# ChainSafe/lumenos

Measured on AMD Instinct MI355X. Metric: prove_eval_seconds_16384x4096, lower is better.
Workload: dtype u64; 1 GPU; Encode+Commit+InnerProduct(r,b)+QueryCols 16384x4096 LogN=14 L=12 K=2 rhoInv=2 queries=309; parallelism=1 GPU: the whole job resident in HBM

## Files before the change

### lumenos_amd/csrc/lm_common.h

```cpp
#pragma once
#include <hip/hip_runtime.h>

#include <algorithm>
#include <cstdarg>
#include <cstdint>
#include <cstdio>
#include <map>
#include <memory>
#include <mutex>
#include <set>
#include <string>
#include <utility>
#include <vector>

#include "../../include/lumenos_hip.h"
#include "lm_arith.h"
#include "lm_dev.h"

#define LM_MAX_LIMBS LUMEN_MAX_LIMBS

struct lm_modmap {
    uint32_t period;
    uint8_t idx[LM_MAX_LIMBS];
};

struct lm_mods {
    mod_t m[LM_MAX_LIMBS];
};

struct lm_prof_entry {
    double total_ms = 0;
    uint64_t launches = 0;
    uint64_t units = 0;
};

struct lm_galois_key {
    lm_dev<u64> d_key;
    lm_dev<uint32_t> d_index;
    lm_dev<uint32_t> d_inv_index;
};

struct lumen_set {
    uint32_t count = 0;
    uint32_t nl = 0;
    uint32_t logw = 0;
    u64 *d = nullptr;
    size_t words = 0;
    bool owner = true;
    lumen_ctx *home = nullptr;
};

struct lm_shared {
    std::recursive_mutex mu;
    lm_dev<tw_t> tw_fwd;
    lm_dev<tw_t> tw_inv;
    std::vector<uint64_t> roots;
    uint32_t fieldN = 0;
    lm_dev<tw_t> scal;
    std::map<uint64_t, lm_galois_key> gkeys;
    std::map<std::string, std::shared_ptr<void>> ext;
};

struct lm_tuning {
    uint32_t ks_batch = 64;
    uint32_t ks_lanes = 0;
    int32_t ks_fused_digits = -1;
    uint32_t debug = 0;
    uint32_t modup_tgroup = 3, moddown_tgroup = 1;
    uint32_t ks_placement = 6;
    uint32_t batch_chunks = 0;
    uint32_t rccl_shared_device = 0;
};

struct lumen_ctx {
    lm_tuning tune;
    std::recursive_mutex mu;
    std::shared_ptr<lm_shared> sh;
    int device = 0;
    hipStream_t stream = nullptr;
    hipStream_t stream2 = nullptr;
    hipEvent_t ev_fork = nullptr, ev_join = nullptr;
    hipStream_t stream_aux = nullptr;
    hipEvent_t ev_aux = nullptr;
    hipEvent_t ev_xdep = nullptr;
    uint32_t aux_digests = 0;
    const u64 *aux_lo = nullptr, *aux_hi = nullptr;
    uint8_t *aux_host = nullptr;
    size_t aux_host_cap = 0;
    void *stage_host = nullptr;
    size_t stage_cap = 0;
    hipEvent_t ev_stage = nullptr;
    void *io_host[2] = {nullptr, nullptr};
    hipEvent_t ev_io[2] = {nullptr, nullptr};
    uint32_t logN = 0, N = 0, L = 0, K = 0;
    uint64_t T = 0;
    uint64_t mod[LM_MAX_LIMBS] = {0};
    uint64_t psi[LM_MAX_LIMBS] = {0};
    lm_mods mods;
    tw_t ninv[LM_MAX_LIMBS];
    std::vector<uint64_t> &roots;
    uint32_t &fieldN;
    std::map<uint64_t, lm_galois_key> &gkeys;
    std::map<std::string, std::shared_ptr<void>> &ext;
    uint64_t mul_counter = 0;
    std::map<std::string, lm_dev<unsigned char>> scratch;
    struct pool_block {
        void *p;
        hipEvent_t ready;
    };
    std::multimap<size_t, pool_block> pool;
    size_t pool_bytes = 0;
    std::set<const void *> lds_attr_done;
    bool prof = false;
    std::map<std::string, lm_prof_entry> prof_tab;
    struct pending_ev {
        std::string name;
        hipEvent_t a, b;
        uint64_t units;
    };
    std::vector<pending_ev> prof_pending;
    std::vector<hipEvent_t> ev_pool;
    hipEvent_t tm0 = nullptr, tm1 = nullptr;
    std::string err;
    explicit lumen_ctx(std::shared_ptr<lm_shared> s)
        : sh(std::move(s)), roots(sh->roots), fieldN(sh->fieldN), gkeys(sh->gkeys), ext(sh->ext) {}
};

static inline size_t lm_ctw(const lumen_ctx *ctx, const lumen_set *s);
#define LM_FULL_WIDTH(ctx, set, what) \
    LM_CHECK(ctx, (set)->logw == 0, "%s: lane-sharded set (1/%u of every limb) where a full-width set is required", what, 1u << (set)->logw)

#define LM_ENTER(ctx)                                             \
    std::lock_guard<std::recursive_mutex> lm_lock_((ctx)->mu);    \
    (void)hipSetDevice((ctx)->device);                            \
    (void)hipGetLastError()
#define LM_SHARED_LOCK(ctx) std::lock_guard<std::recursive_mutex> lm_shlock_((ctx)->sh->mu)

template <class T>
static inline std::shared_ptr<T> lm_ext_get(lumen_ctx *ctx, const std::string &key) {
    LM_SHARED_LOCK(ctx);
    auto it = ctx->ext.find(key);
    return it == ctx->ext.end() ? std::shared_ptr<T>() : std::static_pointer_cast<T>(it->second);
}
static inline void lm_ext_put(lumen_ctx *ctx, const std::string &key, std::shared_ptr<void> v) {
    LM_SHARED_LOCK(ctx);
    ctx->ext[key] = std::move(v);
}

static inline size_t lm_ctw(const lumen_ctx *ctx, const lumen_set *s) { return (size_t)2 * s->nl * (ctx->N >> s->logw); }
// ... 22 lines not shown

template <class... P, class... A>
static inline int lm_launch_flat(lumen_ctx *ctx, void (*kernel)(P...), size_t threads, A &&...args) {
    hipLaunchKernelGGL(kernel, dim3((uint32_t)((threads + 255) / 256)), dim3(256), 0, ctx->stream, std::forward<A>(args)...);
    LM_HIP(ctx, hipGetLastError());
    return 0;
}

struct lm_set_guard {
    lumen_ctx *ctx;
    lumen_set *s;
    lm_set_guard(lumen_ctx *c, lumen_set *x) : ctx(c), s(x) {}
    ~lm_set_guard() {
        if (s) lumen_set_destroy(ctx, s);
    }
    lumen_set *release() {
        lumen_set *r = s;
        s = nullptr;
        return r;
    }
    lm_set_guard(const lm_set_guard &) = delete;
    lm_set_guard &operator=(const lm_set_guard &) = delete;
};

void lm_set_release_async(lumen_ctx *ctx, lumen_set *set);

void *lm_scratch(lumen_ctx *ctx, const char *name, size_t bytes);
void lm_scratch_adopt(lumen_ctx *ctx, const char *name, void *p, size_t bytes);

struct lm_prof_scope {
    lumen_ctx *ctx;
    const char *name;
    uint64_t units;
    hipEvent_t a = nullptr;
    lm_prof_scope(lumen_ctx *c, const char *n, uint64_t u);
    ~lm_prof_scope();
};
void lm_prof_resolve(lumen_ctx *ctx);

static inline uint64_t h_mulmod(uint64_t a, uint64_t b, uint64_t q) {
    return (uint64_t)(((u128)a * b) % q);
}
static inline uint64_t h_powmod(uint64_t a, uint64_t e, uint64_t q) {
    uint64_t r = 1 % q;
    a %= q;
    while (e) {
        if (e & 1) r = h_mulmod(r, a, q);
        a = h_mulmod(a, a, q);
        e >>= 1;
    }
    return r;
}
static inline uint64_t h_invmod(uint64_t a, uint64_t q) { return h_powmod(a, q - 2, q); }
static inline tw_t h_tw(uint64_t w, uint64_t q) {
    tw_t t;
    t.w = w;
    t.wp = (u64)((((u128)w) << 64) / q);
    return t;
}
static inline uint64_t h_r64_mod(uint64_t q) { return (uint64_t)((((u128)1) << 64) % q); }
static inline uint64_t h_p_mod(const lumen_ctx *ctx, uint64_t q) {
    uint64_t P = 1 % q;
    for (uint32_t a = 0; a < ctx->K; a++) P = h_mulmod(P, ctx->mod[ctx->L + a] % q, q);
    return P;
}
static inline uint32_t h_bitrev(uint32_t x, int bits) {
    uint32_t r = 0;
    for (int i = 0; i < bits; i++) r = (r << 1) | ((x >> i) & 1);
    return r;
}

int lm_launch_ntt(lumen_ctx *ctx, u64 *d, uint32_t npoly, const lm_modmap &map, bool inverse);
struct lm_ninv_t;
int lm_launch_ntt_strided(lumen_ctx *ctx, const u64 *src, size_t src_poly_stride, u64 *dst,
                          size_t dst_poly_stride, uint32_t npoly, const lm_modmap &map, bool inverse,
                          const char *prof_name, const lm_ninv_t *inv_scale = nullptr);
int lm_launch_ntt_subring(lumen_ctx *ctx, uint32_t logn, const tw_t *tw, tw_t ninv_scale, const u64 *src,
                          size_t src_poly_stride, u64 *dst, size_t dst_poly_stride, uint32_t npoly,
                          uint32_t mod_idx, bool inverse, const mod_t *explicit_mod = nullptr);
mod_t lm_make_mod(uint64_t q);
void lm_build_tw(uint64_t q, uint64_t psi, uint32_t logN, std::vector<tw_t> &fwd, std::vector<tw_t> &inv);
int lm_rescale_polys(lumen_ctx *ctx, const u64 *src, uint32_t nl, u64 *dst, uint32_t target,
                     uint32_t npoly, u64 *work, u64 *tbuf);
lm_modmap lm_map_q(uint32_t nl);
lm_modmap lm_map_p(const lumen_ctx *ctx);
int lm_encode_dev(lumen_ctx *ctx, const lumen_set *matrix, const u64 *dzero, uint32_t rho_inv, lumen_set **encoded);
hipEvent_t lm_ev_get(lumen_ctx *ctx);
```

### lumenos_amd/csrc/lm_ctx.hip

```cpp
#include <cstring>
#include <thread>

#include "lm_ntt_dev.h"

thread_local std::string lm_global_err;

int lm_fail(lumen_ctx *ctx, const char *fmt, ...) {
    char buf[1024];
    va_list ap;
    va_start(ap, fmt);
    vsnprintf(buf, sizeof(buf), fmt, ap);
    va_end(ap);
    if (ctx) ctx->err = buf;
    lm_global_err = buf;
    fprintf(stderr, "[lumenos_hip] error: %s\n", buf);
    return 1;
}

void *lm_scratch(lumen_ctx *ctx, const char *name, size_t bytes) {
    auto &e = ctx->scratch[name];
    if (e && e.count() >= bytes) return e.get();
    if (e) lm_sync_all(ctx);
    return e.alloc(ctx, bytes, name) ? nullptr : e.get();
}
// ... 71 lines not shown
        }
        ctx->ev_pool.push_back(p.a);
        ctx->ev_pool.push_back(p.b);
    }
    ctx->prof_pending.clear();
}

lm_modmap lm_map_q(uint32_t nl) {
    lm_modmap m;
    m.period = nl;
    for (uint32_t i = 0; i < LM_MAX_LIMBS; i++) m.idx[i] = (uint8_t)(i < nl ? i : 0);
    return m;
}

lm_modmap lm_map_p(const lumen_ctx *ctx) {
    lm_modmap m;
    m.period = ctx->K;
    for (uint32_t i = 0; i < LM_MAX_LIMBS; i++) m.idx[i] = (uint8_t)(ctx->L + (i < ctx->K ? i : 0));
    return m;
}

mod_t lm_make_mod(uint64_t q) {
    mod_t m;
    m.q = q;
    m.qinv64 = (u64)((((u128)1) << 64) / q);
    u64 inv = 1;
    for (int it = 0; it < 6; it++) inv *= 2 - (u64)q * inv;
    m.qneg = (u64)0 - inv;
    u64 r = h_r64_mod(q);
    m.r2 = h_mulmod(r, r, q);
    return m;
}

void lm_build_tw(uint64_t q, uint64_t psi, uint32_t logN, std::vector<tw_t> &fwd, std::vector<tw_t> &inv) {
    uint32_t N = 1u << logN;
    fwd.resize(N);
    inv.resize(N);
    uint64_t psi_inv = h_invmod(psi, q), cf = 1, cb = 1;
    for (uint32_t j = 0; j < N; j++) {
        uint32_t r = h_bitrev(j, (int)logN);
        fwd[r] = h_tw(cf, q);
        inv[r] = h_tw(cb, q);
        cf = h_mulmod(cf, psi, q);
        cb = h_mulmod(cb, psi_inv, q);
    }
}

static void pool_drain(lumen_ctx *ctx) {
    for (auto &kv : ctx->pool) {
        hipFree(kv.second.p);
        if (kv.second.ready) ctx->ev_pool.push_back(kv.second.ready);
    }
    ctx->pool.clear();
    ctx->pool_bytes = 0;
}

static int ctx_private_init(lumen_ctx *ctx) {
    LM_HIP(ctx, hipSetDevice(ctx->device));
    LM_HIP(ctx, hipStreamCreate(&ctx->stream));
    LM_HIP(ctx, hipStreamCreate(&ctx->stream2));
    LM_HIP(ctx, hipEventCreateWithFlags(&ctx->ev_fork, hipEventDisableTiming));
    LM_HIP(ctx, hipEventCreateWithFlags(&ctx->ev_join, hipEventDisableTiming));
    LM_HIP(ctx, hipStreamCreate(&ctx->stream_aux));
    LM_HIP(ctx, hipEventCreateWithFlags(&ctx->ev_aux, hipEventDisableTiming));
    LM_HIP(ctx, hipEventCreateWithFlags(&ctx->ev_stage, hipEventDisableTiming));
    LM_HIP(ctx, hipEventCreateWithFlags(&ctx->ev_xdep, hipEventDisableTiming));
    LM_HIP(ctx, hipEventCreate(&ctx->tm0));
    LM_HIP(ctx, hipEventCreate(&ctx->tm1));
    return 0;
}

static int tuning_set(lm_tuning &t, const char *name, long v) {
    const std::string n(name ? name : "");
    auto in = [&](long lo, long hi) { return v >= lo && v <= hi; };
    if (n == "LUMEN_KS_BATCH") {
        if (!in(1, 4096)) return 2;
        t.ks_batch = (uint32_t)v;
    } else if (n == "LUMEN_KS_LANES") {
        if (!in(0, 2)) return 2;
        t.ks_lanes = (uint32_t)v;
    } else if (n == "LUMEN_KS_FUSED_DIGITS") {
        if (v > LM_MAX_LIMBS) return 2;
        t.ks_fused_digits = v >= 0 ? (int32_t)v : -1;
    } else if (n == "LUMEN_DEBUG") {
        t.debug = v != 0;
    } else if (n == "LUMEN_MODUP_TGROUP") {
        if (!in(1, 31)) return 2;
        t.modup_tgroup = (uint32_t)v;
    } else if (n == "LUMEN_MODDOWN_TGROUP") {
        if (!in(1, 31)) return 2;
        t.moddown_tgroup = (uint32_t)v;
    } else if (n == "LUMEN_KS_PLACEMENT") {
        if (!in(0, 32)) return 2;
        t.ks_placement = (uint32_t)v;
    } else if (n == "LUMEN_BATCH_CHUNKS") {
        if (!in(0, 4096)) return 2;
        t.batch_chunks = (uint32_t)v;
    } else {
        return 1;
    }
    return 0;
}
static void tuning_from_env(lm_tuning &t) {
    for (const char *n : {"LUMEN_KS_BATCH", "LUMEN_KS_LANES", "LUMEN_KS_FUSED_DIGITS", "LUMEN_DEBUG",
                          "LUMEN_MODUP_TGROUP", "LUMEN_MODDOWN_TGROUP", "LUMEN_KS_PLACEMENT", "LUMEN_BATCH_CHUNKS"}) {
        const char *e = getenv(n);
        if (e && *e && tuning_set(t, n, atol(e)))
            fprintf(stderr, "[lumenos_hip] %s=%s is out of range: ignored\n", n, e);
    }
}

extern "C" int lumen_ctx_set_tuning(lumen_ctx *ctx, const char *name, long value) {
    LM_CHECK(nullptr, ctx && name, "lumen_ctx_set_tuning: NULL argument");
    LM_ENTER(ctx);
    const int rc = tuning_set(ctx->tune, name, value);
    LM_CHECK(ctx, rc != 1, "unknown tuning switch %s", name);
    LM_CHECK(ctx, rc == 0, "tuning switch %s: value %ld is out of range (nothing changed)", name, value);
    return 0;
}

extern "C" int lumen_test_allow_shared_device_rccl(lumen_ctx *ctx, int on) {
    LM_CHECK(nullptr, ctx, "lumen_test_allow_shared_device_rccl: NULL ctx");
    LM_ENTER(ctx);
    ctx->tune.rccl_shared_device = on != 0;
    return 0;
}

extern "C" int lumen_ctx_wait(lumen_ctx *ctx, lumen_ctx *other) {
    LM_CHECK(nullptr, ctx && other, "lumen_ctx_wait: NULL argument");
    if (ctx == other) return 0;
    hipEvent_t ev;
    {
        LM_ENTER(other);
        LM_HIP(other, hipEventRecord(other->ev_xdep, other->stream));
        ev = other->ev_xdep;
    }
    LM_ENTER(ctx);
    LM_CHECK(ctx, ctx->device == other->device, "lumen_ctx_wait: contexts on devices %d and %d", ctx->device, other->device);
    LM_HIP(ctx, hipStreamWaitEvent(ctx->stream, ev, 0));
    return 0;
}

extern "C" int lumen_ctx_create(const lumen_params_desc *desc, lumen_ctx **out) {
    if (!desc || !out) return lm_fail(nullptr, "lumen_ctx_create: NULL argument");
    *out = nullptr;
    LM_CHECK(nullptr, desc->abi_version == LUMEN_ABI_VERSION, "ABI version mismatch: got %u want %u",
             desc->abi_version, LUMEN_ABI_VERSION);
    LM_CHECK(nullptr, lm_logn_supported(desc->log_n),
             "log_n %u unsupported: kernels are instantiated for N = 2^8 and 2^10..2^14", desc->log_n);
    LM_CHECK(nullptr, desc->num_q >= 1 && desc->num_q + desc->num_p <= LM_MAX_LIMBS,
             "bad limb counts L=%u K=%u", desc->num_q, desc->num_p);
    int ndev = 0;
    if (hipGetDeviceCount(&ndev) != hipSuccess || ndev == 0)
        return lm_fail(nullptr, "no HIP device visible: the lumenos HIP path has no CPU fallback");
    LM_CHECK(nullptr, desc->device >= 0 && desc->device < ndev, "device %d out of range (have %d)",
             desc->device, ndev);
    std::unique_ptr<lumen_ctx, void (*)(lumen_ctx *)> guard(new lumen_ctx(std::make_shared<lm_shared>()),
                                                            lumen_ctx_destroy);
    lumen_ctx *ctx = guard.get();
    tuning_from_env(ctx->tune);
    ctx->device = desc->device;
    ctx->logN = desc->log_n;
    ctx->N = 1u << desc->log_n;
    ctx->L = desc->num_q;
    ctx->K = desc->num_p;
    ctx->T = desc->plaintext_modulus;
    uint32_t LK = ctx->L + ctx->K, N = ctx->N;
    uint64_t two_n = 2ull * N;
    for (uint32_t i = 0; i < LK; i++) {
        uint64_t q = desc->moduli[i], psi = desc->psi[i];
        static_assert(3 * 0 + 8 >= 8, "the modulus bound (3 log_n + 8) q < 2^64 must imply 8 q < 2^64");
        const uint64_t qmax = UINT64_MAX / (3ull * desc->log_n + 8);
        if (q < (1ull << 20) || q > qmax || (q & (two_n - 1)) != 1)
            return lm_fail(nullptr, "modulus %u (%llu) must be == 1 mod 2N and below %llu", i,
                           (unsigned long long)q, (unsigned long long)qmax);
        if (h_powmod(psi, N, q) != q - 1)
            return lm_fail(nullptr, "psi[%u] is not a primitive 2N-th root of unity", i);
        ctx->mod[i] = q;
        ctx->psi[i] = psi;
        ctx->mods.m[i] = lm_make_mod(q);
        ctx->ninv[i] = h_tw(h_invmod(N % q, q), q);
    }
    for (uint32_t i = LK; i < LM_MAX_LIMBS; i++) ctx->mods.m[i] = ctx->mods.m[0];
    if (int rc = ctx_private_init(ctx)) return rc;
    std::vector<tw_t> f, b, fwd, inv;
    for (uint32_t i = 0; i < LK; i++) {
        lm_build_tw(ctx->mod[i], ctx->psi[i], ctx->logN, f, b);
// ... 469 lines not shown
```

### lumenos_amd/csrc/lm_keyswitch.hip

```cpp
#include <cstdlib>
#include <cstring>

#include "lm_ks_host.h"

uint32_t ks_batch(const lumen_ctx *ctx) { return ctx->tune.ks_batch; }

uint32_t ks_lanes(const lumen_ctx *ctx) {
    return ctx->tune.ks_lanes ? ctx->tune.ks_lanes : (ctx->logN <= 13 ? 2 : 1);
}

int check_level_of_chain(lumen_ctx *ctx, const lumen_set *in, const char *what) {
    LM_FULL_WIDTH(ctx, in, what);
    LM_CHECK(ctx, in->nl >= 1 && in->nl <= ctx->L, "%s: set has %u limbs, the chain has %u", what, in->nl, ctx->L);
    return 0;
}

__device__ __forceinline__ u32 bx_v(u128 A, u128 M, u64 y0, u64 y1, u64 m0, u64 m1) {
    const u128 D1 = A >= M ? A - M : M - A, D2 = 2 * M - A;
    if ((u64)(D1 >> 64) >= 8 && (u64)(D2 >> 64) >= 8) return A >= M ? 1u : 0u;
    double vf = 0.0;
    vf += (double)y0 / (double)m0;
    vf += (double)y1 / (double)m1;
    return (u32)(u64)vf;
}
// ... 565 lines not shown
    return 0;
}

static int modup_work_list(lumen_ctx *ctx, KsTables *tb, uint32_t B, const uint32_t **out) {
    const uint32_t LM_MODUP_TGROUP = ctx->tune.modup_tgroup;
    LM_SHARED_LOCK(ctx);
    LM_CHECK(ctx, B >= 1 && B <= 65535 && tb->beta <= 255 && tb->nl + ctx->K <= 255,
             "key-switch batch of %u columns (beta %u) does not fit the packed work list", B, tb->beta);
    const uint32_t cache_key = B | (LM_MODUP_TGROUP << 16);
    auto it = tb->d_work.find(cache_key);
    if (it != tb->d_work.end()) {
        *out = it->second.get();
        return 0;
    }
    const uint32_t LK = tb->nl + ctx->K, beta = tb->beta;
    std::vector<std::vector<uint8_t>> need(beta);
    for (uint16_t pr : tb->pairs) need[pr & 0xFF].push_back((uint8_t)(pr >> 8));
    std::vector<std::vector<uint32_t>> lists(8);
    for (uint32_t x = 0; x < 8; x++)
        for (uint32_t t0 = 0; t0 < LK; t0 += LM_MODUP_TGROUP)
            for (uint32_t b = x; b < B; b += 8)
                for (uint32_t d = 0; d < beta; d++)
                    for (uint8_t t : need[d])
                        if (t >= t0 && t < t0 + LM_MODUP_TGROUP) lists[x].push_back(b | (d << 16) | ((uint32_t)t << 24));
    return interleave_work_lists(ctx, lists, (size_t)B * tb->pairs.size(), "extension", tb->d_work, cache_key, out);
}

static int moddown_work_list(lumen_ctx *ctx, KsTables *tb, uint32_t B, const uint32_t **out) {
    const uint32_t LM_MODDOWN_TGROUP = ctx->tune.moddown_tgroup;
    LM_SHARED_LOCK(ctx);
    LM_CHECK(ctx, B >= 1 && 2 * (uint64_t)B <= 65535, "key-switch batch of %u columns does not fit the packed work list", B);
    const uint32_t cache_key = B | (LM_MODDOWN_TGROUP << 17);
    auto it = tb->d_work_down.find(cache_key);
    if (it != tb->d_work_down.end()) {
        *out = it->second.get();
        return 0;
    }
    const uint32_t L = tb->nl;
    std::vector<std::vector<uint32_t>> lists(8);
    for (uint32_t x = 0; x < 8; x++)
        for (uint32_t t0 = 0; t0 < L; t0 += LM_MODDOWN_TGROUP)
            for (uint32_t pw = x; pw < 2 * B; pw += 8)
                for (uint32_t t = t0; t < std::min<uint32_t>(t0 + LM_MODDOWN_TGROUP, L); t++) lists[x].push_back(pw | (t << 16));
    return interleave_work_lists(ctx, lists, (size_t)2 * B * L, "ModDown", tb->d_work_down, cache_key, out);
}

template <int LOGN>
static uint32_t intt_pack_slots(lumen_ctx *ctx) {
    static const uint32_t v = [&] {
        hipDeviceProp_t prop;
        int per_cu = 0;
        if (hipGetDeviceProperties(&prop, ctx->device) != hipSuccess) return 256u;
        (void)hipFuncSetAttribute(reinterpret_cast<const void *>(&k_intt_pack<LOGN>),
                                  hipFuncAttributeMaxDynamicSharedMemorySize, 160 * 1024);
        constexpr lm_geom g = lm_geom_lds(LOGN);
        if (hipOccupancyMaxActiveBlocksPerMultiprocessor(&per_cu, k_intt_pack<LOGN>, g.threads, g.lds) != hipSuccess || per_cu < 1) {
            per_cu = (int)std::max<size_t>(1, std::min<size_t>(160 * 1024 / g.lds, 2048 / g.threads));
        }
        (void)hipGetLastError();
        if (ctx->tune.debug)
            fprintf(stderr, "[lumenos_hip] k_intt_pack<%d>: %d workgroup(s) per CU, %d CUs\n", LOGN, per_cu,
                    prop.multiProcessorCount);
        return (uint32_t)prop.multiProcessorCount * (uint32_t)per_cu;
    }();
    return v;
}
static uint32_t ks_fused_digits(lumen_ctx *ctx, uint32_t B, uint32_t L) {
    const long forced = ctx->tune.ks_fused_digits;
    const uint32_t pairs = L / 2;
    if (forced >= 0) return std::min<uint32_t>((uint32_t)forced, pairs);
    uint32_t slots = 0;
    if (lm_for_logn(ctx, ctx->logN, [&](auto n) { return slots = intt_pack_slots<n>(ctx), 0; })) return 0;
    for (uint32_t nf = pairs; nf >= 1; nf--)
        if (((uint64_t)B * nf) % slots == 0) return nf;
    return 0;
}

static dim3 ks_mac_grid(const lumen_ctx *ctx, uint32_t B, uint32_t L) {
    return dim3(((ctx->N / LM_MAC_VEC + 255) / 256) * (L + ctx->K) * ((B + LM_MAC_COLS - 1) / LM_MAC_COLS));
}

}

int rotate_accumulate(lumen_ctx *ctx, const u64 *acc, u64 *acc_out, uint32_t B, const lm_galois_key &gk,
                      KsTables *tb, const KsScratch &s) {
    const uint32_t N = ctx->N, L = tb->nl, K = ctx->K, beta = tb->beta;
    const uint32_t pshift = ctx->L - L, key_beta = (ctx->L + K - 1) / K;
    const uint32_t nf = K == 2 ? ks_fused_digits(ctx, B, L) : 0;
    if (nf) {
        const uint32_t grid = B * nf + B * (L - 2 * nf);
        lm_prof_scope ps(ctx, "ks_intt_c1", (uint64_t)B * L);
        if (int rc = lm_for_logn(ctx, ctx->logN, [&](auto n) {
                return lm_launch(ctx, k_intt_pack<n>, lm_geom_lds(n), grid, acc, s.coef, B, L, nf, ctx->mods, tb->yscale,
                                 ctx->sh->tw_inv.get());
            }))
            return rc;
    } else {
        if (int rc = lm_launch_ntt_strided(ctx, acc + (size_t)L * N, (size_t)2 * L * N, s.coef, (size_t)L * N, B,
                                           lm_map_q(L), true, "ks_intt_c1", &tb->yscale))
            return rc;
    }
    if (K == 2 && nf < beta) {
        lm_prof_scope ps(ctx, "ks_pack_v", (uint64_t)B);
        hipLaunchKernelGGL(k_pack_v, dim3(2048), dim3(256), 0, ctx->stream, s.coef + (size_t)2 * nf * N, (size_t)L * N,
                           B, beta - nf, K, 2 * nf, L - 2 * nf, ctx->logN, ctx->mods);
        LM_HIP(ctx, hipGetLastError());
    }
    {
        const uint64_t nb = (uint64_t)B * tb->pairs.size();
        const uint32_t *work = nullptr;
        if (int rc = modup_work_list(ctx, tb, B, &work)) return rc;
        lm_prof_scope ps(ctx, "ks_modup_ntt", nb);
        if (int rc = lm_for_logn(ctx, ctx->logN, [&](auto n) {
                return lm_launch(ctx, k_modup_ntt<n>, lm_geom_fwd(n), (uint32_t)nb, s.coef, acc, s.ext, tb->d_bx.get(), B, L, K, beta,
                                 pshift, work, ctx->mods, ctx->sh->tw_fwd.get());
            }))
            return rc;
    }
    {
        lm_prof_scope ps(ctx, "ks_mac", (uint64_t)B);
        hipLaunchKernelGGL(k_ks_mac, ks_mac_grid(ctx, B, L), dim3(256), 0, ctx->stream, s.ext, acc, gk.d_key.get(), s.u, B, L, K,
                           beta, pshift, key_beta, ctx->logN, ctx->mods);
        LM_HIP(ctx, hipGetLastError());
    }
    {
        u64 *up = s.u + ks_u_at(0, L, B, L, K) * N;
        const size_t pstride = (size_t)K * N;
        if (int rc = lm_launch_ntt_strided(ctx, up, pstride, up, pstride, B * 2, lm_map_p(ctx), true, "ks_intt_p",
                                           &tb->yscale))
            return rc;
        if (K == 2) {
            lm_prof_scope ps(ctx, "ks_pack_v", (uint64_t)B);
            hipLaunchKernelGGL(k_pack_v, dim3(2048), dim3(256), 0, ctx->stream, up, pstride, B * 2, 1u, K, ctx->L, K,
                               ctx->logN, ctx->mods);
            LM_HIP(ctx, hipGetLastError());
        }
    }
    {
        const uint32_t *work_down = nullptr;
        if (int rc = moddown_work_list(ctx, tb, B, &work_down)) return rc;
        lm_prof_scope ps(ctx, "ks_moddown_ntt", (uint64_t)B * 2 * L);
        return lm_for_logn(ctx, ctx->logN, [&](auto n) {
            return lm_launch(ctx, k_moddown_ntt<n>, lm_geom_fwd(n), B * 2 * L, s.u, acc, acc_out, tb->d_bxp.get(), tb->d_pinv.get(),
                             gk.d_index.get(), gk.d_inv_index.get(), work_down, B, L, K, ctx->mods, ctx->sh->tw_fwd.get());
        });
    }
}

namespace {

int inner_sum_batch(lumen_ctx *ctx, u64 *acc, uint32_t B, uint32_t n, KsTables *tb, const KsScratch &s) {
    uint64_t gal[64];
    const uint32_t cnt = lumen_inner_sum_galois_elements(ctx, n, gal);
    for (uint32_t r = 0; r < cnt; r++) {
        const lm_galois_key *gk;
        {
            LM_SHARED_LOCK(ctx);
            auto it = ctx->gkeys.find(gal[r]);
            LM_CHECK(ctx, it != ctx->gkeys.end(), "Galois key for element %llu not loaded",
                     (unsigned long long)gal[r]);
            gk = &it->second;
        }
        u64 *src = (r & 1) ? s.acc2 : acc, *dst = (r & 1) ? acc : s.acc2;
        if (int rc = rotate_accumulate(ctx, src, dst, B, *gk, tb, s)) return rc;
    }
    if (cnt & 1)
        LM_HIP(ctx, hipMemcpyAsync(acc, s.acc2, (size_t)B * 2 * tb->nl * ctx->N * 8, hipMemcpyDeviceToDevice,
                                   ctx->stream));
    return 0;
}

}

extern "C" int lumen_ks_mac_probe(lumen_ctx *ctx, uint32_t batch, const void *ext, const void *acc, const void *key,
                                  void *u, uint32_t reps, float *ms_per_launch) {
    LM_CHECK(nullptr, ctx && ms_per_launch, "lumen_ks_mac_probe: NULL argument");
    LM_ENTER(ctx);
    KsTables *tb = nullptr;
    if (int rc = get_tables(ctx, &tb)) return rc;
    const uint32_t N = ctx->N, L = ctx->L, K = ctx->K, B = batch ? batch : ks_batch(ctx);
    LM_CHECK(ctx, B <= 65535 && reps >= 1 && reps <= 100000, "lumen_ks_mac_probe: batch %u / reps %u out of range", B, reps);
    KsScratch s;
    if (int rc = get_scratch(ctx, B, tb, &s)) return rc;
    if (!acc) acc = lm_scratch(ctx, "ks_acc", (size_t)B * 2 * L * N * 8);
    if (!acc) return 1;
    if (!key) {
        LM_SHARED_LOCK(ctx);
        LM_CHECK(ctx, !ctx->gkeys.empty(), "lumen_ks_mac_probe: no Galois key loaded");
        key = ctx->gkeys.begin()->second.d_key.get();
    }
    const u64 *pe = ext ? (const u64 *)ext : s.ext;
    u64 *pu = u ? (u64 *)u : s.u;
    const dim3 grid = ks_mac_grid(ctx, B, L);
    auto launch = [&] {
        hipLaunchKernelGGL(k_ks_mac, grid, dim3(256), 0, ctx->stream, pe, (const u64 *)acc, (const u64 *)key, pu, B, L, K,
                           tb->beta, 0u, tb->beta, ctx->logN, ctx->mods);
    };
    for (int i = 0; i < 3; i++) launch();
    LM_HIP(ctx, hipGetLastError());
    LM_HIP(ctx, hipEventRecord(ctx->tm0, ctx->stream));
    for (uint32_t i = 0; i < reps; i++) launch();
    LM_HIP(ctx, hipGetLastError());
    LM_HIP(ctx, hipEventRecord(ctx->tm1, ctx->stream));
    LM_HIP(ctx, hipEventSynchronize(ctx->tm1));
    float ms = 0;
    LM_HIP(ctx, hipEventElapsedTime(&ms, ctx->tm0, ctx->tm1));
    *ms_per_launch = ms / (float)reps;
    return 0;
}

static int check_inner_sum_level(lumen_ctx *ctx, const lumen_set *in, const char *what) {
    LM_FULL_WIDTH(ctx, in, what);
    LM_CHECK(ctx, in->nl == ctx->L, "%s is implemented at the top level only (set has %u of %u limbs)", what,
             in->nl, ctx->L);
    return 0;
}

namespace {

int inner_sum_at(lumen_ctx *ctx, const lumen_set *in, uint32_t n, lumen_set **out) {
    LM_CHECK(ctx, n && !(n & (n - 1)) && n <= ctx->N, "InnerSum length %u is not a power of two <= N", n);
    KsTables *top = nullptr, *tb = nullptr;
    if (int rc = get_tables(ctx, &top)) return rc;
    if (int rc = get_tables_at(ctx, in->nl, &tb)) return rc;
    lumen_set *o = nullptr;
    if (int rc = lumen_set_create(ctx, in->count, in->nl, &o)) return rc;
    lm_set_guard og(ctx, o);
    if (in->words)
        LM_HIP(ctx, hipMemcpyAsync(o->d, in->d, in->words * 8, hipMemcpyDeviceToDevice, ctx->stream));
    const uint32_t Bmax = std::min<uint32_t>(ks_batch(ctx), std::max(in->count, 1u));
    KsScratch s;
    if (int rc = get_scratch(ctx, Bmax, top, &s)) return rc;
    const size_t ctw = (size_t)2 * in->nl * ctx->N;
    for (uint32_t first = 0; first < in->count; first += Bmax) {
        const uint32_t B = std::min(Bmax, in->count - first);
        if (int rc = inner_sum_batch(ctx, o->d + (size_t)first * ctw, B, n, tb, s)) return rc;
    }
    if (int rc = acc_canon(ctx, o->d, o->words, in->nl)) return rc;
    *out = og.release();
    return 0;
}

int matrix_inner_sum_at(lumen_ctx *ctx, const lumen_set *matrix, const uint64_t *pt, uint32_t rows, lumen_set **out) {
    LM_CHECK(ctx, rows && !(rows & (rows - 1)) && rows <= ctx->N, "rows=%u is not a power of two <= N", rows);
    KsTables *top = nullptr, *tb = nullptr;
    if (int rc = get_tables(ctx, &top)) return rc;
    if (int rc = get_tables_at(ctx, matrix->nl, &tb)) return rc;
    u64 *ptT = nullptr;
    if (int rc = upload_ptT(ctx, pt, matrix->nl, &ptT)) return rc;
    const uint32_t N = ctx->N, L = matrix->nl;
    const uint32_t target = std::min<uint32_t>(2, L);
    lumen_set *o = nullptr;
    if (int rc = lumen_set_create(ctx, matrix->count, target, &o)) return rc;
    lm_set_guard og(ctx, o);
    const uint32_t Bmax = std::min<uint32_t>(ks_batch(ctx), std::max(matrix->count, 1u));
    const uint32_t group = std::min<uint32_t>(8 * Bmax, std::max(matrix->count, 1u));
    KsScratch s[2];
    const size_t ctw = (size_t)2 * L * N, octw = (size_t)2 * target * N;
    const size_t group_bytes = (size_t)group * 2 * ctx->L * N * 8;
    u64 *acc = nullptr;
    if (get_scratch(ctx, Bmax, top, &s[0], 0, &acc, group_bytes) || (ks_lanes(ctx) > 1 && get_scratch(ctx, Bmax, top, &s[1], 1)))
        return 1;
    u64 *work = (u64 *)lm_scratch(ctx, "rescale_work", group_bytes);
    u64 *tbuf = (u64 *)lm_scratch(ctx, "rescale_t", (size_t)group * 2 * N * 8);
    if (!acc || !work || !tbuf) return 1;
    for (uint32_t g0 = 0; g0 < matrix->count; g0 += group) {
        const uint32_t gn = std::min(group, matrix->count - g0);
        if (ks_lanes(ctx) > 1) {
            LM_HIP(ctx, hipEventRecord(ctx->ev_fork, ctx->stream));
            LM_HIP(ctx, hipStreamWaitEvent(ctx->stream2, ctx->ev_fork, 0));
        }
        uint32_t lane = 0;
        for (uint32_t first = 0; first < gn; first += Bmax, lane = (lane + 1) % ks_lanes(ctx)) {
            const uint32_t B = std::min(Bmax, gn - first);
            u64 *a = acc + (size_t)first * ctw;
            LaneGuard guard(ctx, (int)lane);
            if (int rc = launch_mul_plain(ctx, matrix->d + (size_t)(g0 + first) * ctw, a, ptT, (size_t)B * ctw, L, B))
                return rc;
            if (int rc = inner_sum_batch(ctx, a, B, rows, tb, s[lane])) return rc;
        }
        if (ks_lanes(ctx) > 1) {
            LM_HIP(ctx, hipEventRecord(ctx->ev_join, ctx->stream2));
            LM_HIP(ctx, hipStreamWaitEvent(ctx->stream, ctx->ev_join, 0));
        }
        if (L > target) {
            if (int rc = lm_rescale_polys(ctx, acc, L, o->d + (size_t)g0 * octw, target, gn * 2, work, tbuf)) return rc;
        } else {
            if (int rc = acc_canon(ctx, acc, (size_t)gn * ctw, L)) return rc;
            LM_HIP(ctx, hipMemcpyAsync(o->d + (size_t)g0 * octw, acc, (size_t)gn * ctw * 8, hipMemcpyDeviceToDevice,
                                       ctx->stream));
        }
    }
    *out = og.release();
    return 0;
}

}

extern "C" int lumen_inner_sum(lumen_ctx *ctx, const lumen_set *in, uint32_t n, lumen_set **out) {
    LM_CHECK(nullptr, ctx && in && out, "lumen_inner_sum: NULL argument");
    LM_ENTER(ctx);
    if (int rc = check_inner_sum_level(ctx, in, "InnerSum")) return rc;
    return inner_sum_at(ctx, in, n, out);
}

extern "C" int lumen_inner_sum_at_level(lumen_ctx *ctx, const lumen_set *in, uint32_t n, lumen_set **out) {
    LM_CHECK(nullptr, ctx && in && out, "lumen_inner_sum_at_level: NULL argument");
    LM_ENTER(ctx);
    if (int rc = check_level_of_chain(ctx, in, "InnerSum")) return rc;
    return inner_sum_at(ctx, in, n, out);
}

extern "C" int lumen_matrix_inner_sum(lumen_ctx *ctx, const lumen_set *matrix, const uint64_t *pt,
                                      uint32_t rows, lumen_set **out) {
    LM_CHECK(nullptr, ctx && matrix && pt && out, "lumen_matrix_inner_sum: NULL argument");
    LM_ENTER(ctx);
    if (int rc = check_inner_sum_level(ctx, matrix, "matrixInnerSumEval")) return rc;
    return matrix_inner_sum_at(ctx, matrix, pt, rows, out);
}

extern "C" int lumen_matrix_inner_sum_at_level(lumen_ctx *ctx, const lumen_set *matrix, const uint64_t *pt,
                                               uint32_t rows, lumen_set **out) {
    LM_CHECK(nullptr, ctx && matrix && pt && out, "lumen_matrix_inner_sum_at_level: NULL argument");
    LM_ENTER(ctx);
    if (int rc = check_level_of_chain(ctx, matrix, "matrixInnerSumEval")) return rc;
    return matrix_inner_sum_at(ctx, matrix, pt, rows, out);
}
```

### lumenos_amd/csrc/lm_ks_host.h

```cpp
#pragma once
#include "lm_ks_dev.h"

struct KsTables {
    lm_dev<bx_t> d_bx;
    lm_dev<bx_t> d_bxp;
    lm_dev<tw_t> d_pinv;
    uint32_t nl = 0;
    uint32_t beta = 0;
    lm_ninv_t yscale;
    std::vector<uint16_t> pairs;
    std::map<uint32_t, lm_dev<uint32_t>> d_work;
    std::map<uint32_t, lm_dev<uint32_t>> d_work_down;
};
int get_tables(lumen_ctx *ctx, KsTables **out);
int get_tables_at(lumen_ctx *ctx, uint32_t nl, KsTables **out);

struct KsScratch {
    u64 *coef, *ext, *u, *acc2;
};

int rotate_accumulate(lumen_ctx *ctx, const u64 *acc, u64 *acc_out, uint32_t B, const lm_galois_key &gk,
                      KsTables *tb, const KsScratch &s);
int get_scratch(lumen_ctx *ctx, uint32_t B, KsTables *tb, KsScratch *s, int lane = 0, u64 **group_acc = nullptr,
                size_t group_acc_bytes = 0);

int upload_ptT(lumen_ctx *ctx, const uint64_t *pt, uint32_t nl, u64 **out);
int launch_mul_plain(lumen_ctx *ctx, const u64 *ct, u64 *out, const u64 *ptT, size_t words, uint32_t nl,
                     uint32_t ncts);

std::shared_ptr<lm_galois_key> lm_relin_key(lumen_ctx *ctx);
int check_level_of_chain(lumen_ctx *ctx, const lumen_set *in, const char *what);
uint32_t ks_batch(const lumen_ctx *ctx);
uint32_t ks_lanes(const lumen_ctx *ctx);
struct LaneGuard {
    lumen_ctx *ctx;
    hipStream_t saved;
    LaneGuard(lumen_ctx *c, int lane) : ctx(c), saved(c->stream) {
        if (lane) ctx->stream = ctx->stream2;
    }
    ~LaneGuard() { ctx->stream = saved; }
};
```

### lumenos_amd/csrc/lm_rescale.hip

```cpp
#include "lm_ntt_dev.h"

struct rescale_consts {
    u64 half;
    u64 half_mod[LM_MAX_LIMBS];
    tw_t qlinv[LM_MAX_LIMBS];
};

template <int LOGN>
__global__ LM_GEOM_BOUNDS(lm_geom_lds(LOGN)) void k_rescale_last(const u64 *__restrict__ src, size_t src_poly_stride,
                                                       uint32_t last, u64 *__restrict__ tbuf, mod_t md,
                                                       tw_t ninv, u64 half, const tw_t *__restrict__ tw) {
    extern __shared__ __attribute__((aligned(16))) u64 sm[];
    constexpr uint32_t N = 1u << LOGN;
    const uint32_t tid = threadIdx.x;
    const lm_qc c = lm_make_qc(md);
    const u64 *p = src + (size_t)blockIdx.x * src_poly_stride + (size_t)last * N;
    u64 *o = tbuf + (size_t)blockIdx.x * N;
    auto ld = [&](uint32_t i0, u64 *v, int count) { lm_load_run(p, i0, v, count); };
    auto st = [&](uint32_t i, u64 v) { o[i] = lm_addmod(lm_shoup_cs(v, ninv, c.q, c.nq), half, c.q); };
    lm_ntt_inverse<LOGN>(sm, tw, c, tid, ld, st);
}

template <int LOGN>
__global__ LM_GEOM_BOUNDS(lm_geom_lds(LOGN)) void k_rescale_limb(const u64 *src, size_t src_poly_stride, u64 *dst,
// ... 16 lines not shown
        lm_load_run(cin, i0, cv, count);
#pragma unroll
        for (int k = 0; k < 8; k++)
            if (k < count) r[k] = lm_shoup_cs(lm_submod(cv[k], lm_reduce_s(v[k], c.q, c.nq, c.qinv64), c.q), qlinv, c.q, c.nq);
        lm_store_run(o, i0, r, count);
    };
    lm_ntt_forward<LOGN>(sm, tw_all + (size_t)limb * N, c, tid, ld, st);
}

struct rs_step_t {
    u64 k;
    u64 pad;
    tw_t inv;
};
struct rs_half_t {
    u64 h[LM_MAX_LIMBS];
};
struct RescaleTables {
    lm_dev<rs_step_t> d_steps;
    rs_half_t half;
};

static int get_rescale_tables(lumen_ctx *ctx, RescaleTables **out) {
    LM_SHARED_LOCK(ctx);
    auto it = ctx->ext.find("rescale_tables");
    if (it != ctx->ext.end()) {
        *out = static_cast<RescaleTables *>(it->second.get());
        return 0;
    }
    auto sp = std::make_shared<RescaleTables>();
    std::vector<rs_step_t> steps((size_t)LM_MAX_LIMBS * LM_MAX_LIMBS);
    memset(steps.data(), 0, steps.size() * sizeof(rs_step_t));
    for (uint32_t l = 0; l < LM_MAX_LIMBS; l++) {
        const uint64_t ql = ctx->mod[l < ctx->L ? l : 0], half = (ql - 1) >> 1;
        sp->half.h[l] = half;
        for (uint32_t j = 0; j < l && l < ctx->L; j++) {
            const uint64_t qj = ctx->mod[j];
            rs_step_t &e = steps[(size_t)l * LM_MAX_LIMBS + j];
            const uint64_t M = ql / qj + 1;
            if (M > 16) return 2;
            e.k = half + M * qj;
            e.inv = h_tw(h_invmod(ql % qj, qj), qj);
        }
    }
    if (int rc = sp->d_steps.upload(ctx, steps, "the rescale tables")) return rc;
    ctx->ext["rescale_tables"] = sp;
    *out = sp.get();
    return 0;
}

__global__ __launch_bounds__(256) void k_rescale_coef(const u64 *__restrict__ coef, size_t src_poly_stride,
                                                      u64 *__restrict__ dst, size_t dst_poly_stride, uint32_t nl,
                                                      uint32_t target, uint32_t logN, size_t total, lm_mods mods,
                                                      const rs_step_t *__restrict__ steps, rs_half_t half) {
    const size_t idx = (size_t)blockIdx.x * blockDim.x + threadIdx.x;
    if (idx >= total) return;
    const size_t poly = idx >> logN, i = idx & (((size_t)1 << logN) - 1);
    const u64 *p = coef + poly * src_poly_stride + i;
    u64 c[LM_MAX_LIMBS];
#pragma unroll
    for (int j = 0; j < LM_MAX_LIMBS; j++) c[j] = (uint32_t)j < nl ? p[(size_t)j << logN] : 0;
#pragma unroll
    for (int l = LM_MAX_LIMBS - 1; l >= 1; l--) {
        if ((uint32_t)l < nl && (uint32_t)l >= target) {
            const u64 ql = mods.m[l].q;
            u64 t = lm_csub(lm_csub(c[l], 2 * ql), ql);
            t = lm_addmod(t, half.h[l], ql);
#pragma unroll
            for (int j = 0; j < l; j++) {
                const rs_step_t e = steps[l * LM_MAX_LIMBS + j];
                c[j] = lm_shoup3<true>(c[j] + e.k - t, e.inv.w, e.inv.wp, 0 - mods.m[j].q);
            }
        }
    }
    u64 *o = dst + poly * dst_poly_stride + i;
#pragma unroll
    for (int j = 0; j < LM_MAX_LIMBS; j++)
        if ((uint32_t)j < target) {
            const u64 qj = mods.m[j].q;
            o[(size_t)j << logN] = lm_csub(lm_csub(c[j], 2 * qj), qj);
        }
}

static int rescale_polys_coef(lumen_ctx *ctx, const u64 *src, uint32_t nl, u64 *dst, uint32_t target, uint32_t npoly,
                              u64 *work) {
    RescaleTables *tb = nullptr;
    if (int rc = get_rescale_tables(ctx, &tb)) return rc;
    const uint32_t N = ctx->N;
    if (int rc = lm_launch_ntt_strided(ctx, src, (size_t)nl * N, work, (size_t)nl * N, npoly, lm_map_q(nl), true,
                                       "rescale_intt", nullptr))
        return rc;
    {
        lm_prof_scope ps(ctx, "rescale_coef", npoly);
        const size_t total = (size_t)npoly * N;
        hipLaunchKernelGGL(k_rescale_coef, dim3((uint32_t)((total + 255) / 256)), dim3(256), 0, ctx->stream, work,
                           (size_t)nl * N, dst, (size_t)target * N, nl, target, ctx->logN, total, ctx->mods,
                           tb->d_steps.get(), tb->half);
        LM_HIP(ctx, hipGetLastError());
    }
    return lm_launch_ntt_strided(ctx, dst, (size_t)target * N, dst, (size_t)target * N, npoly, lm_map_q(target), false,
                                 "rescale_ntt", nullptr);
}

template <int LOGN>
static int rescale_polys_t(lumen_ctx *ctx, const u64 *src, uint32_t nl, u64 *dst, uint32_t target,
                           uint32_t npoly, u64 *work, u64 *tbuf) {
    if (work && (uint64_t)(nl + target + 1) * (nl - target) / 2 > (uint64_t)nl + target) {
        const int rc = rescale_polys_coef(ctx, src, nl, dst, target, npoly, work);
        if (rc != 2) return rc;
    }
    const uint32_t N = ctx->N;
    const u64 *cur = src;
    for (uint32_t cur_nl = nl; cur_nl > target; cur_nl--) {
        const uint32_t last = cur_nl - 1;
        const bool final_step = cur_nl - 1 == target;
        u64 *out = final_step ? dst : work;
        const size_t out_stride = (size_t)(final_step ? target : nl) * N;
        rescale_consts rc;
        const uint64_t ql = ctx->mod[last];
        rc.half = (ql - 1) >> 1;
        for (uint32_t i = 0; i < LM_MAX_LIMBS; i++) {
            const uint64_t qi = ctx->mod[i < last ? i : 0];
            rc.half_mod[i] = rc.half % qi;
            rc.qlinv[i] = h_tw(h_invmod(ql % qi, qi), qi);
        }
        {
            lm_prof_scope ps(ctx, "rescale_last_intt", npoly);
            if (int e = lm_launch(ctx, k_rescale_last<LOGN>, lm_geom_lds(LOGN), npoly, cur, (size_t)nl * N, last, tbuf,
                                  ctx->mods.m[last], ctx->ninv[last], (u64)rc.half, ctx->sh->tw_inv.get() + (size_t)last * N))
                return e;
        }
        {
            lm_prof_scope ps(ctx, "rescale_limb_ntt", (uint64_t)npoly * last);
            if (int e = lm_launch(ctx, k_rescale_limb<LOGN>, lm_geom_lds(LOGN), npoly * last, cur, (size_t)nl * N, out,
                                  out_stride, tbuf, npoly, ctx->mods, rc, ctx->sh->tw_fwd.get()))
                return e;
        }
        cur = work;
    }
    return 0;
}

int lm_rescale_polys(lumen_ctx *ctx, const u64 *src, uint32_t nl, u64 *dst, uint32_t target,
                     uint32_t npoly, u64 *work, u64 *tbuf) {
    return lm_for_logn(ctx, ctx->logN, [&](auto n) { return rescale_polys_t<n>(ctx, src, nl, dst, target, npoly, work, tbuf); });
}

extern "C" int lumen_rescale(lumen_ctx *ctx, const lumen_set *in, uint32_t target_limbs, lumen_set **out) {
    LM_CHECK(nullptr, ctx && in && out, "lumen_rescale: NULL argument");
    LM_ENTER(ctx);
    LM_FULL_WIDTH(ctx, in, "lumen_rescale");
    LM_CHECK(ctx, target_limbs >= 1 && target_limbs <= in->nl, "target_limbs %u out of range [1,%u]",
             target_limbs, in->nl);
    lumen_set *o = nullptr;
    if (int rc = lumen_set_create(ctx, in->count, target_limbs, &o)) return rc;
    lm_set_guard og(ctx, o);
    const uint32_t N = ctx->N, nl = in->nl;
    const size_t in_ctw = (size_t)2 * nl * N, out_ctw = (size_t)2 * target_limbs * N;
    if (target_limbs == nl) {
        if (in->words)
            LM_HIP(ctx, hipMemcpyAsync(o->d, in->d, in->words * sizeof(u64), hipMemcpyDeviceToDevice, ctx->stream));
        *out = og.release();
        return 0;
    }
    uint32_t chunk = (uint32_t)std::max<size_t>(1, ((size_t)2 << 30) / (in_ctw * sizeof(u64)));
    if (chunk >= 128) chunk -= chunk % 128;
    chunk = std::min(chunk, std::max(in->count, 1u));
    u64 *work = nullptr;
    if (nl - target_limbs > 1) {
        work = (u64 *)lm_scratch(ctx, "rescale_work", (size_t)chunk * in_ctw * sizeof(u64));
        if (!work) return 1;
    }
    u64 *tbuf = (u64 *)lm_scratch(ctx, "rescale_t", (size_t)chunk * 2 * N * sizeof(u64));
    if (!tbuf) return 1;
    for (uint32_t first = 0; first < in->count; first += chunk) {
        const uint32_t n = std::min(chunk, in->count - first);
        if (int rc = lm_rescale_polys(ctx, in->d + (size_t)first * in_ctw, nl, o->d + (size_t)first * out_ctw,
                                      target_limbs, n * 2, work, tbuf))
            return rc;
    }
    *out = og.release();
    return 0;
}
```

Baseline: 1.701 s.

## Fuse final inner-sum rotation moddown with rescale inverse NTT

Adds a k_ks_close kernel that takes the last rotation of each inner-sum batch and, in one pass, performs the moddown, the Galois automorphism, the accumulate and the inverse NTT, writing coefficient-domain output straight into the rescale work buffer. The rescale then starts from coefficients and skips its own inverse-NTT pass. This removes a separate moddown kernel and a full read/write of the accumulator per batch. In exchange the fused kernel does gathered loads through the automorphism index, and the change adds a tuning switch (LUMEN_KS_CLOSE_FUSED, on by default).

Result: faster. 1.684 s, median of 6 (-1.0%).

```diff
diff --git a/lumenos_amd/csrc/lm_common.h b/lumenos_amd/csrc/lm_common.h
--- a/lumenos_amd/csrc/lm_common.h
+++ b/lumenos_amd/csrc/lm_common.h
@@ -65,6 +65,7 @@
     uint32_t ks_batch = 64;
     uint32_t ks_lanes = 0;
     int32_t ks_fused_digits = -1;
+    uint32_t ks_close_fused = 1;
     uint32_t debug = 0;
     uint32_t modup_tgroup = 3, moddown_tgroup = 1;
     uint32_t ks_placement = 6;
@@ -253,6 +254,8 @@
 void lm_build_tw(uint64_t q, uint64_t psi, uint32_t logN, std::vector<tw_t> &fwd, std::vector<tw_t> &inv);
 int lm_rescale_polys(lumen_ctx *ctx, const u64 *src, uint32_t nl, u64 *dst, uint32_t target,
                      uint32_t npoly, u64 *work, u64 *tbuf);
+int lm_rescale_coef_ready(lumen_ctx *ctx);
+int lm_rescale_polys_from_coef(lumen_ctx *ctx, const u64 *coef, uint32_t nl, u64 *dst, uint32_t target, uint32_t npoly);
 lm_modmap lm_map_q(uint32_t nl);
 lm_modmap lm_map_p(const lumen_ctx *ctx);
 int lm_encode_dev(lumen_ctx *ctx, const lumen_set *matrix, const u64 *dzero, uint32_t rho_inv, lumen_set **encoded);
diff --git a/lumenos_amd/csrc/lm_ctx.hip b/lumenos_amd/csrc/lm_ctx.hip
--- a/lumenos_amd/csrc/lm_ctx.hip
+++ b/lumenos_amd/csrc/lm_ctx.hip
@@ -177,6 +177,9 @@
     } else if (n == "LUMEN_KS_FUSED_DIGITS") {
         if (v > LM_MAX_LIMBS) return 2;
         t.ks_fused_digits = v >= 0 ? (int32_t)v : -1;
+    } else if (n == "LUMEN_KS_CLOSE_FUSED") {
+        if (!in(0, 1)) return 2;
+        t.ks_close_fused = (uint32_t)v;
     } else if (n == "LUMEN_DEBUG") {
         t.debug = v != 0;
     } else if (n == "LUMEN_MODUP_TGROUP") {
@@ -197,7 +200,7 @@
     return 0;
 }
 static void tuning_from_env(lm_tuning &t) {
-    for (const char *n : {"LUMEN_KS_BATCH", "LUMEN_KS_LANES", "LUMEN_KS_FUSED_DIGITS", "LUMEN_DEBUG",
+    for (const char *n : {"LUMEN_KS_BATCH", "LUMEN_KS_LANES", "LUMEN_KS_FUSED_DIGITS", "LUMEN_KS_CLOSE_FUSED", "LUMEN_DEBUG",
                           "LUMEN_MODUP_TGROUP", "LUMEN_MODDOWN_TGROUP", "LUMEN_KS_PLACEMENT", "LUMEN_BATCH_CHUNKS"}) {
         const char *e = getenv(n);
         if (e && *e && tuning_set(t, n, atol(e)))
diff --git a/lumenos_amd/csrc/lm_keyswitch.hip b/lumenos_amd/csrc/lm_keyswitch.hip
--- a/lumenos_amd/csrc/lm_keyswitch.hip
+++ b/lumenos_amd/csrc/lm_keyswitch.hip
@@ -671,8 +671,8 @@
 
 }
 
-int rotate_accumulate(lumen_ctx *ctx, const u64 *acc, u64 *acc_out, uint32_t B, const lm_galois_key &gk,
-                      KsTables *tb, const KsScratch &s) {
+static int rotate_front(lumen_ctx *ctx, const u64 *acc, uint32_t B, const lm_galois_key &gk, KsTables *tb,
+                        const KsScratch &s) {
     const uint32_t N = ctx->N, L = tb->nl, K = ctx->K, beta = tb->beta;
     const uint32_t pshift = ctx->L - L, key_beta = (ctx->L + K - 1) / K;
     const uint32_t nf = K == 2 ? ks_fused_digits(ctx, B, L) : 0;
@@ -725,6 +725,13 @@
             LM_HIP(ctx, hipGetLastError());
         }
     }
+    return 0;
+}
+
+int rotate_accumulate(lumen_ctx *ctx, const u64 *acc, u64 *acc_out, uint32_t B, const lm_galois_key &gk,
+                      KsTables *tb, const KsScratch &s) {
+    if (int rc = rotate_front(ctx, acc, B, gk, tb, s)) return rc;
+    const uint32_t L = tb->nl, K = ctx->K;
     {
         const uint32_t *work_down = nullptr;
         if (int rc = moddown_work_list(ctx, tb, B, &work_down)) return rc;
@@ -738,9 +745,19 @@
 
 namespace {
 
-int inner_sum_batch(lumen_ctx *ctx, u64 *acc, uint32_t B, uint32_t n, KsTables *tb, const KsScratch &s) {
+int rotate_close(lumen_ctx *ctx, const u64 *acc, u64 *coef_out, uint32_t B, const lm_galois_key &gk, uint64_t gal_el,
+                 KsTables *tb, const KsScratch &s) {
+    if (int rc = rotate_front(ctx, acc, B, gk, tb, s)) return rc;
+    const uint32_t *work_down = nullptr;
+    if (int rc = moddown_work_list(ctx, tb, B, &work_down)) return rc;
+    return ks_close_launch(ctx, acc, coef_out, B, gk, gal_el, tb, s, work_down);
+}
+
+int inner_sum_batch(lumen_ctx *ctx, u64 *acc, uint32_t B, uint32_t n, KsTables *tb, const KsScratch &s,
+                    u64 *close_out = nullptr) {
     uint64_t gal[64];
     const uint32_t cnt = lumen_inner_sum_galois_elements(ctx, n, gal);
+    LM_CHECK(ctx, !close_out || cnt, "InnerSum(%u) has no rotation to close", n);
     for (uint32_t r = 0; r < cnt; r++) {
         const lm_galois_key *gk;
         {
@@ -751,6 +768,8 @@
             gk = &it->second;
         }
         u64 *src = (r & 1) ? s.acc2 : acc, *dst = (r & 1) ? acc : s.acc2;
+        if (close_out && r + 1 == cnt)
+            return rotate_close(ctx, src, close_out, B, *gk, gal[r], tb, s);
         if (int rc = rotate_accumulate(ctx, src, dst, B, *gk, tb, s)) return rc;
     }
     if (cnt & 1)
@@ -853,6 +872,12 @@
     u64 *work = (u64 *)lm_scratch(ctx, "rescale_work", group_bytes);
     u64 *tbuf = (u64 *)lm_scratch(ctx, "rescale_t", (size_t)group * 2 * N * 8);
     if (!acc || !work || !tbuf) return 1;
+    bool close = false;
+    if (L > target && rows > 1 && ctx->tune.ks_close_fused) {
+        const int rc = lm_rescale_coef_ready(ctx);
+        if (rc && rc != 2) return rc;
+        close = rc == 0;
+    }
     for (uint32_t g0 = 0; g0 < matrix->count; g0 += group) {
         const uint32_t gn = std::min(group, matrix->count - g0);
         if (ks_lanes(ctx) > 1) {
@@ -866,13 +891,16 @@
             LaneGuard guard(ctx, (int)lane);
             if (int rc = launch_mul_plain(ctx, matrix->d + (size_t)(g0 + first) * ctw, a, ptT, (size_t)B * ctw, L, B))
                 return rc;
-            if (int rc = inner_sum_batch(ctx, a, B, rows, tb, s[lane])) return rc;
+            if (int rc = inner_sum_batch(ctx, a, B, rows, tb, s[lane], close ? work + (size_t)first * ctw : nullptr))
+                return rc;
         }
         if (ks_lanes(ctx) > 1) {
             LM_HIP(ctx, hipEventRecord(ctx->ev_join, ctx->stream2));
             LM_HIP(ctx, hipStreamWaitEvent(ctx->stream, ctx->ev_join, 0));
         }
-        if (L > target) {
+        if (close) {
+            if (int rc = lm_rescale_polys_from_coef(ctx, work, L, o->d + (size_t)g0 * octw, target, gn * 2)) return rc;
+        } else if (L > target) {
             if (int rc = lm_rescale_polys(ctx, acc, L, o->d + (size_t)g0 * octw, target, gn * 2, work, tbuf)) return rc;
         } else {
             if (int rc = acc_canon(ctx, acc, (size_t)gn * ctw, L)) return rc;
diff --git a/lumenos_amd/csrc/lm_ks_close.hip b/lumenos_amd/csrc/lm_ks_close.hip
--- /dev/null
+++ b/lumenos_amd/csrc/lm_ks_close.hip
@@ -0,0 +1,112 @@
+#include "lm_ks_host.h"
+
+#ifndef LM_KS_CLOSE_PF
+#define LM_KS_CLOSE_PF 4
+#endif
+
+template <int LOGN>
+__global__ LM_GEOM_BOUNDS(lm_geom_lds(LOGN)) void k_ks_close(const u64 *__restrict__ u, const u64 *__restrict__ acc_in,
+                                                              u64 *__restrict__ out, const bx_t *__restrict__ bxp,
+                                                              const tw_t *__restrict__ pinv,
+                                                              const uint32_t *__restrict__ index,
+                                                              const uint32_t *__restrict__ inv_index, uint32_t ginv,
+                                                              const uint32_t *__restrict__ work, uint32_t B, uint32_t L,
+                                                              uint32_t K, lm_mods mods, lm_ninv_t ninv,
+                                                              const tw_t *__restrict__ tw_all) {
+    extern __shared__ __attribute__((aligned(16))) u64 sm[];
+    constexpr uint32_t N = 1u << LOGN;
+    const uint32_t tid = threadIdx.x;
+    const uint32_t wk = work[blockIdx.x];
+    const uint32_t pw = wk & 0xFFFF;
+    const uint32_t t = wk >> 16;
+    const uint32_t w = pw & 1;
+    const bx_t c = bxp[t];
+    const lm_qc qc = lm_make_qc(mods.m[t]);
+    const u64 *up0 = u + ks_u_at(pw, L, B, L, K) * N;
+    const u64 *up1 = c.ns == 2 ? up0 + N : up0;
+    const u64 *uq = u + ks_u_at(pw, t, B, L, K) * N;
+    const u64 *ain = acc_in + ((size_t)pw * L + t) * N;
+    u64 *o = out + ((size_t)pw * L + t) * N;
+    constexpr uint32_t NW = lm_nthreads(LOGN) / 64, BLK = N / NW, IT = BLK / 128, CH = IT < 4 ? IT : 4;
+    static_assert(IT >= 1 && IT % CH == 0, "a wave stages its block as pairs of words, 128 per instruction");
+    {
+        const uint32_t wave = tid >> 6, lane = tid & 63;
+        const uint32_t sb = NW > 1 ? (uint32_t)__builtin_amdgcn_readfirstlane((int)(index[wave * BLK] / BLK)) : 0u;
+#pragma unroll
+        for (uint32_t k0 = 0; k0 < IT; k0 += CH) {
+            uint2 p[CH];
+            ulonglong2 x[CH], c0[CH];
+#pragma unroll
+            for (uint32_t k = 0; k < CH; k++) {
+                const uint32_t s = sb * BLK + 2 * lane + (k0 + k) * 128;
+                p[k] = *reinterpret_cast<const uint2 *>(inv_index + s);
+                x[k] = *reinterpret_cast<const ulonglong2 *>(uq + s);
+                if (w == 0) c0[k] = *reinterpret_cast<const ulonglong2 *>(ain + s);
+            }
+#pragma unroll
+            for (uint32_t k = 0; k < CH; k++) {
+                sm[LM_PAD(wave * BLK + (p[k].x & (BLK - 1)))] = w == 0 ? x[k].x + c0[k].x : x[k].x;
+                sm[LM_PAD(wave * BLK + (p[k].y & (BLK - 1)))] = w == 0 ? x[k].y + c0[k].y : x[k].y;
+            }
+        }
+        lm_wave_sync();
+    }
+    auto ld = [&](uint32_t j0, u64 *v, int count) {
+        lm_load_run(ain, j0, v, count);
+#pragma unroll
+        for (int k = 0; k < 8; k++)
+            if (k < count) {
+                const u64 x = sm[LM_PAD(j0 + k)];
+                v[k] = w == 0 ? lm_csub(v[k] + x, 2 * qc.q) : v[k] + x;
+            }
+    };
+    constexpr int R_LAST = lm_pass_r(LOGN, 0), LOG_T0 = LOGN - R_LAST, CNT = 1 << R_LAST;
+    constexpr int PF = LM_KS_CLOSE_PF < CNT ? LM_KS_CLOSE_PF : CNT;
+    tw_t npi = pinv[t];
+    npi.w = qc.q - npi.w, npi.wp = ~npi.wp;
+    struct close_t {
+        u64 *o;
+        const u64 *up0, *up1;
+        const bx_t &c;
+        const lm_qc &qc;
+        tw_t ni, npi;
+        uint32_t ginv;
+        u64 hi[PF], lo[PF];
+        __device__ __forceinline__ uint32_t src(uint32_t i) const { return (ginv * i) & (2 * N - 1); }
+        __device__ __forceinline__ void fetch(uint32_t i, u64 &h, u64 &l) const {
+            const uint32_t s = src(i) & (N - 1);
+            h = up0[s], l = up1[s];
+        }
+        __device__ __forceinline__ void pre(uint32_t w0) {
+#pragma unroll
+            for (int k = 0; k < PF; k++) fetch(w0 + ((uint32_t)k << LOG_T0), hi[k], lo[k]);
+        }
+        __device__ __forceinline__ void operator()(uint32_t i, u64 v, int k) {
+            const u64 h = hi[k % PF], l = lo[k % PF];
+            if (k + PF < CNT) fetch(i + ((uint32_t)PF << LOG_T0), hi[k % PF], lo[k % PF]);
+            const u64 m = lm_shoup3<true>(bx_apply(c, h, l, qc), npi.w, npi.wp, qc.nq);
+            const u64 r = lm_shoup3<true>(v, ni.w, ni.wp, qc.nq);
+            u64 y = r + (src(i) >= N ? qc.q3 - m : m);
+            y = lm_csub(lm_csub(y, 4 * qc.q), 2 * qc.q);
+            o[i] = lm_csub(y, qc.q);
+        }
+    } st{o, up0, up1, c, qc, ninv.t[t], npi, ginv, {}, {}};
+    lm_ntt_inverse<LOGN>(sm, tw_all + (size_t)t * N, qc, tid, ld, st);
+}
+
+static uint32_t inv_mod_2n(uint64_t g, uint32_t N) {
+    uint64_t x = g;
+    for (int i = 0; i < 5; i++) x *= 2 - g * x;
+    return (uint32_t)(x & (2ull * N - 1));
+}
+
+int ks_close_launch(lumen_ctx *ctx, const u64 *acc, u64 *out, uint32_t B, const lm_galois_key &gk, uint64_t gal_el,
+                    KsTables *tb, const KsScratch &s, const uint32_t *work_down) {
+    const uint32_t L = tb->nl, K = ctx->K;
+    const uint32_t ginv = inv_mod_2n(gal_el, ctx->N);
+    lm_prof_scope ps(ctx, "rescale_intt", (uint64_t)B * 2 * L);
+    return lm_for_logn(ctx, ctx->logN, [&](auto n) {
+        return lm_launch(ctx, k_ks_close<n>, lm_geom_lds(n), B * 2 * L, s.u, acc, out, tb->d_bxp.get(), tb->d_pinv.get(),
+                         gk.d_index.get(), gk.d_inv_index.get(), ginv, work_down, B, L, K, ctx->mods, lm_ninv_of(ctx), ctx->sh->tw_inv.get());
+    });
+}
diff --git a/lumenos_amd/csrc/lm_ks_host.h b/lumenos_amd/csrc/lm_ks_host.h
--- a/lumenos_amd/csrc/lm_ks_host.h
+++ b/lumenos_amd/csrc/lm_ks_host.h
@@ -21,6 +21,8 @@
 
 int rotate_accumulate(lumen_ctx *ctx, const u64 *acc, u64 *acc_out, uint32_t B, const lm_galois_key &gk,
                       KsTables *tb, const KsScratch &s);
+int ks_close_launch(lumen_ctx *ctx, const u64 *acc, u64 *out, uint32_t B, const lm_galois_key &gk, uint64_t gal_el,
+                    KsTables *tb, const KsScratch &s, const uint32_t *work_down);
 int get_scratch(lumen_ctx *ctx, uint32_t B, KsTables *tb, KsScratch *s, int lane = 0, u64 **group_acc = nullptr,
                 size_t group_acc_bytes = 0);
 
diff --git a/lumenos_amd/csrc/lm_rescale.hip b/lumenos_amd/csrc/lm_rescale.hip
--- a/lumenos_amd/csrc/lm_rescale.hip
+++ b/lumenos_amd/csrc/lm_rescale.hip
@@ -122,14 +122,15 @@
         }
 }
 
-static int rescale_polys_coef(lumen_ctx *ctx, const u64 *src, uint32_t nl, u64 *dst, uint32_t target, uint32_t npoly,
-                              u64 *work) {
+int lm_rescale_coef_ready(lumen_ctx *ctx) {
+    RescaleTables *tb = nullptr;
+    return get_rescale_tables(ctx, &tb);
+}
+
+int lm_rescale_polys_from_coef(lumen_ctx *ctx, const u64 *work, uint32_t nl, u64 *dst, uint32_t target, uint32_t npoly) {
     RescaleTables *tb = nullptr;
     if (int rc = get_rescale_tables(ctx, &tb)) return rc;
     const uint32_t N = ctx->N;
-    if (int rc = lm_launch_ntt_strided(ctx, src, (size_t)nl * N, work, (size_t)nl * N, npoly, lm_map_q(nl), true,
-                                       "rescale_intt", nullptr))
-        return rc;
     {
         lm_prof_scope ps(ctx, "rescale_coef", npoly);
         const size_t total = (size_t)npoly * N;
@@ -140,6 +141,16 @@
     }
     return lm_launch_ntt_strided(ctx, dst, (size_t)target * N, dst, (size_t)target * N, npoly, lm_map_q(target), false,
                                  "rescale_ntt", nullptr);
+}
+
+static int rescale_polys_coef(lumen_ctx *ctx, const u64 *src, uint32_t nl, u64 *dst, uint32_t target, uint32_t npoly,
+                              u64 *work) {
+    if (int rc = lm_rescale_coef_ready(ctx)) return rc;
+    const uint32_t N = ctx->N;
+    if (int rc = lm_launch_ntt_strided(ctx, src, (size_t)nl * N, work, (size_t)nl * N, npoly, lm_map_q(nl), true,
+                                       "rescale_intt", nullptr))
+        return rc;
+    return lm_rescale_polys_from_coef(ctx, work, nl, dst, target, npoly);
 }
 
 template <int LOGN>
```
